# scraed/LanPaint

Measured on AMD Instinct MI355X. Metric: langevin_think_iterations_per_sec, higher is better.
Workload: dtype f32; 1 GPU; c2_sdxl: latent 1x4x128x128 per GPU, 30 sigmas x 5 think iterations, 50% box mask, stub backbone x->(0.9x,0.8x), VE/Karras schedule; rng=torch, graph=auto, mask_format=f32, mask_seen_by_kernels=bits, captured_calls=1, backbone_io=f32, replicas=1, rows_per_gpu=1, global_rows=1, latent_elements_per_gpu=65536

## Files before the change

include/lanpaint_hip.h:

```cpp
#ifndef LANPAINT_HIP_H
#define LANPAINT_HIP_H

#include <stdint.h>

#ifdef __cplusplus
extern "C" {
#endif

#define LP_ABI_VERSION 25

#define LP_API __attribute__((visibility("default")))

#define LP_OK             0
#define LP_E_INVALID     -1
#define LP_E_UNSUPPORTED -2
#define LP_E_LAUNCH      -3
#define LP_E_ALIGN       -4

#define LP_COEF_STRIDE   36
#define LP_C_SCALE        0
#define LP_C_SQRT_ABT     1
#define LP_C_OMA          2
#define LP_C_ABT          3
#define LP_C_RSIGMA       4
// ... 146 lines not shown
    int32_t      es_n_steps;
    int32_t      es_reset;
    const float* sg_sigma;
    const float* sg_schedule;
    float*       sg_times_out;
    float*       sg_scalars_out;
    int32_t*     sg_seq_out;
    uint64_t*    sg_valid_out;
    double       sg_min_step_frac;
    int32_t      sg_schedule_len, sg_seq, sg_n_steps, sg_early_stop, sg_total_steps, sg_guess;
    double*      clk_out;
    const void*  av_bits;
    float        av_frac;
    uint32_t     reserved2;
    float*       es_xte;
    uint32_t     tune;
    uint32_t     io_valid;
} lp_step_desc;
#define LP_TUNE_VEC1          (1u << 0)
#define LP_TUNE_VEC4          (1u << 1)
#define LP_TUNE_ES_NO_DECIDE  (1u << 2)
#define LP_TUNE_ES_NO_FOLD    (1u << 3)
#define LP_TUNE_ES_NO_ATOMICS (1u << 4)
#define LP_CLK_STAMPS 9

typedef struct lp_final_desc {
    int64_t   n_el;
    uint32_t  flags;
    float     cfg_scale;
    const void*  model_out;
    const void*  uncond;
    const float* y;
    const void*  mask;
    const float* x_src;
    float*       x_dst;
    float*       out;
    uint64_t*    rng_bump_ptr;
    uint64_t     rng_bump;
    const uint64_t* io_table;
} lp_final_desc;

LP_API int lp_abi_version(void);
LP_API const char* lp_strerror(int code);

LP_API int lp_coeffs(const lp_hyper* hyper, const float* ve_sigma, int ve_stride, const float* abt, int abt_stride,
              const float* replace_sigma, int rs_stride, const float* step_override, int step_stride,
              const float* t_model, int t_stride, int rows, float* coef_table, void* stream);
// ... 386 lines not shown
```

lanpaint_amd/csrc/cabi.hip:

```cpp
#include <cmath>

#include "lp_common.h"

namespace lp {
int step_dispatch(const lp_step_desc* d, hipStream_t stream, void* timer);
int replace_node_update(const lp_step_desc* d, hipGraphExec_t exec, const lp_graph_binding* b);
int timer_create(void** out);
int timer_destroy(void* h);
int timer_elapsed_ns(void* h, double* ns);
int coeffs_dispatch(const lp_hyper* h, const float* ve, int ve_stride, const float* abt, int abt_stride,
                    const float* rs, int rs_stride, const float* step_ov, int step_stride, const float* t_model,
                    int t_stride, int rows, float* table, hipStream_t stream);
int finalize_dispatch(const lp_final_desc* d, hipStream_t stream);
int sigma_times_dispatch(const float* sigma, int rows, const float* schedule, int schedule_len, int is_flow, float* times,
                         float* scalars, int32_t* seq_out, int32_t seq, hipStream_t stream);
int sigma_times_rule_dispatch(const float* sigma, int rows, const float* schedule, int schedule_len, int is_flow,
                              float* times, float* scalars, int32_t* seq_out, int32_t seq, int32_t n_steps, int32_t early_stop,
                              int32_t total_steps, double min_step_frac, int32_t guess, uint64_t* valid_out, hipStream_t stream);
int blend_dispatch(const lp_blend_desc* d, hipStream_t stream);
int philox_dispatch(float* out, int64_t n_el, uint64_t seed, uint64_t offset, uint32_t slot, hipStream_t stream);
int ring_dispatch(const float* mask, float* ring, int64_t planes, int height, int width, hipStream_t stream);
int wmse_dispatch(const float* a, const float* b, const float* mask, const float* ring, int64_t n_el, double* acc,
                  double* scratch, int scratch_blocks, hipStream_t stream);
int torch_normal_dispatch(float* out, int64_t n, uint64_t seed, uint64_t offset, uint32_t bg, hipStream_t stream);
// ... 178 lines not shown
        if (!c->graph_exec) return LP_E_INVALID;
        rc = lp::replace_node_update(c->replace, static_cast<hipGraphExec_t>(c->graph_exec), c->replace_binding);
    } else if (c->replace) {
        rc = lp::step_dispatch(c->replace, s, nullptr);
    }
    if (rc != LP_OK) return rc;
    if (c->graph_exec && hipGraphLaunch(static_cast<hipGraphExec_t>(c->graph_exec), s) != hipSuccess) return LP_E_LAUNCH;
    return c->final ? lp::finalize_dispatch(c->final, s) : LP_OK;
}

int lp_graph_bind_replace(void* graph, const lp_step_desc* captured, lp_graph_binding* out) {
    if (!graph || !captured || !out) return LP_E_INVALID;
    hipGraph_t g = static_cast<hipGraph_t>(graph);
    size_t n_root = 0;
    if (hipGraphGetRootNodes(g, nullptr, &n_root) != hipSuccess || n_root != 1) return LP_E_UNSUPPORTED;
    hipGraphNode_t root = nullptr;
    if (hipGraphGetRootNodes(g, &root, &n_root) != hipSuccess || !root) return LP_E_UNSUPPORTED;
    hipGraphNodeType ty;
    if (hipGraphNodeGetType(root, &ty) != hipSuccess || ty != hipGraphNodeTypeKernel) return LP_E_UNSUPPORTED;
    hipKernelNodeParams p{};
    if (hipGraphKernelNodeGetParams(root, &p) != hipSuccess || !p.func || !p.kernelParams) return LP_E_UNSUPPORTED;
    void* const* kp = p.kernelParams;
    const lp_step_desc* dn = static_cast<const lp_step_desc*>(kp[8]);
    if (*static_cast<void* const*>(kp[0]) != captured->x_t || *static_cast<const void* const*>(kp[2]) != captured->x ||
        !dn || dn->phases != captured->phases || !(dn->phases & LP_PH_REPLACE) || dn->n_el != captured->n_el)
        return LP_E_UNSUPPORTED;
    lp::StepPlan plan;
    const int rc = lp::plan_step(*captured, &plan);
    if (rc != LP_OK) return rc;
    if (!lp::plan_is_node(plan, p.func, p.gridDim, p.blockDim)) return LP_E_UNSUPPORTED;
    out->node = root; out->func = p.func;
    out->grid[0] = p.gridDim.x; out->grid[1] = p.gridDim.y; out->grid[2] = p.gridDim.z;
    out->block[0] = p.blockDim.x; out->block[1] = p.blockDim.y; out->block[2] = p.blockDim.z;
    out->shared_bytes = p.sharedMemBytes; out->reserved0 = 0;
    return LP_OK;
}

int lp_graph_clone_tail(void* graph, void** tail_graph_out, void** tail_exec_out) {
    if (!graph || !tail_graph_out || !tail_exec_out) return LP_E_INVALID;
    hipGraph_t clone = nullptr;
    if (hipGraphClone(&clone, static_cast<hipGraph_t>(graph)) != hipSuccess) return LP_E_LAUNCH;
    size_t n_root = 0;
    hipGraphNode_t root = nullptr;
    hipGraphExec_t exec = nullptr;
    if (hipGraphGetRootNodes(clone, nullptr, &n_root) == hipSuccess && n_root == 1 &&
        hipGraphGetRootNodes(clone, &root, &n_root) == hipSuccess && root && hipGraphDestroyNode(root) == hipSuccess &&
        hipGraphInstantiate(&exec, clone, nullptr, nullptr, 0) == hipSuccess) {
        *tail_graph_out = clone; *tail_exec_out = exec;
// ... 220 lines not shown
```

lanpaint_amd/csrc/lp_common.h:

```cpp
#pragma once
#include <hip/hip_runtime.h>
#include <hip/hip_ext.h>
#include <stdint.h>

#include "lanpaint_hip.h"

namespace lp {

constexpr int kWave = 64;

__device__ __forceinline__ int nearest_exact_index(int i, int in_size, int out_size, int rule) {
#pragma clang fp contract(off)
    const float scale = static_cast<float>(in_size) / static_cast<float>(out_size);
    const float at = static_cast<float>(i) + 0.5f;
    int s;
    if (rule == LP_NN_ATEN_SCALAR) {
        s = static_cast<int>(floorf(at * scale));
    } else {
        float src = (rule == LP_NN_ATEN_CPU_GENERIC_FMA) ? __builtin_fmaf(scale, at, -0.5f) : (scale * at - 0.5f);
        src = src < 0.0f ? 0.0f : src;
        s = static_cast<int>(floorf(static_cast<float>(static_cast<double>(src) + 0.5)));
    }
    return s < in_size - 1 ? s : in_size - 1;
}
// ... 417 lines not shown
        c[LP_C_RSCALE] = static_cast<float>(1.0 / static_cast<double>(c[LP_C_SCALE]));
    }
    const double oma_d = static_cast<double>(oma);
    float* q = c + (g ? LP_C_REGION1 : LP_C_REGION0);
    const double a = (g ? static_cast<double>(h.one_plus_lambda) : 1.0) / oma_d;
    const double dt = static_cast<double>(g ? dty : dtx);
    const double tau = s ? dt * 0.5 : dt;
    const double e = exp(-a * tau);
    const double k = -expm1(-a * tau) / a;
    const double k2 = -expm1(-2.0 * a * tau) / (2.0 * a);
    const double sd = sqrt(fmax(2.0 * k2, 0.0));
    q[s ? LP_R_E_HALF : LP_R_E_FULL] = static_cast<float>(e);
    q[s ? LP_R_K_HALF : LP_R_K_FULL] = static_cast<float>(k);
    q[s ? LP_R_STD_HALF : LP_R_STD_FULL] = static_cast<float>(sd);
    if (s == 0) {
        const double cx0 = sqrt(static_cast<double>(abt_f)) / oma_d;
        q[LP_R_DT] = static_cast<float>(dt);
        q[LP_R_A] = static_cast<float>(a);
        q[LP_R_CX0] = static_cast<float>(cx0);
        q[LP_R_CXT] = g ? static_cast<float>(a - 1.0 / oma_d) : 0.0f;
    }
}

__device__ __forceinline__ double wave_sum(double v) {
#pragma unroll
    for (int off = kWave / 2; off > 0; off >>= 1) v += __shfl_down(v, off, kWave);
    return v;
}

template <int CTRL, int ROW_MASK>
__device__ __forceinline__ float dpp_move(float v) {
    return __builtin_bit_cast(float, __builtin_amdgcn_update_dpp(0, __builtin_bit_cast(int, v), CTRL, ROW_MASK, 0xf, false));
}
template <int CTRL, int ROW_MASK>
__device__ __forceinline__ double dpp_move(double v) {
    const long long b = __builtin_bit_cast(long long, v);
    const int lo = __builtin_amdgcn_update_dpp(0, static_cast<int>(b), CTRL, ROW_MASK, 0xf, false);
    const int hi = __builtin_amdgcn_update_dpp(0, static_cast<int>(b >> 32), CTRL, ROW_MASK, 0xf, false);
    return __builtin_bit_cast(double, (static_cast<long long>(hi) << 32) | static_cast<long long>(static_cast<uint32_t>(lo)));
}
template <int CTRL, int ROW_MASK, typename T, int N>
__device__ __forceinline__ void dpp_level(T (&v)[N]) {
    T t[N];
#pragma unroll
    for (int k = 0; k < N; ++k) t[k] = dpp_move<CTRL, ROW_MASK>(v[k]);
#pragma unroll
// ... 110 lines not shown
    if (min_step_frac <= 0.0 || frac >= min_step_frac || n_steps <= 0) return n_steps;
    const double r = rint(static_cast<double>(n_steps) * frac / min_step_frac);
    return r > 0.0 ? static_cast<int32_t>(r) : 0;
}

__host__ __device__ inline int x0_dtype(uint32_t flags) {
    return (flags & LP_FL_X0_BF16) ? DT_BF16 : (flags & LP_FL_X0_F16) ? DT_F16 : DT_F32;
}
__host__ __device__ inline int xin_dtype(uint32_t flags) {
    return (flags & LP_FL_XIN_BF16) ? DT_BF16 : (flags & LP_FL_XIN_F16) ? DT_F16 : DT_F32;
}

struct StepPlan {
    const void* kernel;
    dim3 grid;
    uint32_t ph_ct;
    int vec;
    bool decide;
    int decide_slot;
    int mode, x0w, rng, es;
    bool st;
};
struct StepArgs {
    void* x_t;
    void* C;
    const void *a2, *a3, *a4, *a5;
    int32_t el_per_row;
    uint32_t flags;
    void* ptr[9];
};
int plan_step(const lp_step_desc& d, StepPlan* out, bool timed = false);
void pack_step_args(const StepPlan& p, const lp_step_desc& d, StepArgs* a);
bool plan_is_node(const StepPlan& p, const void* func, const dim3& grid, const dim3& block);

}
```

lanpaint_amd/csrc/step_kernel.hip:

```cpp
#include <cstddef>

#include "lp_common.h"

#pragma clang fp contract(off)

namespace lp {

struct RegionCoef {
    float e_full, k_full, std_full, e_half, k_half, std_half, dt, a, cx0, cxt;
};

struct RowCoef {
    float scale, sqrt_abt, oma, abt, rsigma, dtx, dty, ax, ay, dx, dy, valid;
    RegionCoef reg[2];
    float rscale;
};

__device__ __forceinline__ RowCoef load_row(const float* __restrict__ coef, int row) {
    const float* c = coef + static_cast<int64_t>(row) * LP_COEF_STRIDE;
    RowCoef r;
    r.scale = c[LP_C_SCALE]; r.sqrt_abt = c[LP_C_SQRT_ABT]; r.oma = c[LP_C_OMA]; r.abt = c[LP_C_ABT];
    r.rsigma = c[LP_C_RSIGMA]; r.dtx = c[LP_C_DTX]; r.dty = c[LP_C_DTY]; r.ax = c[LP_C_AX]; r.ay = c[LP_C_AY];
    r.dx = c[LP_C_DX]; r.dy = c[LP_C_DY]; r.valid = c[LP_C_VALID];
    r.rscale = c[LP_C_RSCALE];
// ... 212 lines not shown
    return t;
}
__device__ __forceinline__ uint64_t clk_after_loads() {
    uint64_t t;
    asm volatile("s_waitcnt vmcnt(0)\n s_memtime %0\n s_waitcnt lgkmcnt(0)" : "=s"(t)::"memory");
    return t;
}
__device__ __forceinline__ uint64_t clk_real() {
    uint64_t t;
    asm volatile("s_memrealtime %0\n s_waitcnt lgkmcnt(0)" : "=s"(t)::"memory");
    return t;
}
#define LP_CLK_DECL                                                                                                  \
    uint64_t clk_t[LP_CLK_STAMPS] = {}, clk_r0 = 0;                                                                  \
    const bool clk_on = d_arg.clk_out && threadIdx.x == 0 && blockIdx.y == 0 && (blockIdx.x == 0 || blockIdx.x == gridDim.x - 1); \
    if (clk_on) { clk_t[0] = clk_now(); clk_r0 = clk_real(); }
#define LP_CLK(k) if (clk_on) clk_t[k] = clk_now();
__device__ __forceinline__ uint64_t clk_when(uint32_t a, uint32_t b) {
    uint64_t t;
    asm volatile("s_memtime %0\n s_waitcnt lgkmcnt(0)" : "=s"(t) : "s"(a), "s"(b) : "memory");
    return t;
}
#define LP_CLK_WHEN(k, a, b) if (clk_on) clk_t[k] = clk_when(a, b);
#define LP_CLK_LOADS(k) if (clk_on) clk_t[k] = clk_after_loads();
#define LP_CLK_FLUSH                                                                                                 \
    if (clk_on) {                                                                                                    \
        double* clk_o = d_arg.clk_out + (blockIdx.x == 0 ? 0 : 16);                                                  \
        for (int k = 0; k < LP_CLK_STAMPS; ++k) clk_o[k] = clk_t[k] ? static_cast<double>(clk_t[k] - clk_t[0]) : 0.0; \
        clk_o[15] = static_cast<double>(clk_real() - clk_r0);                                                        \
        clk_o[14] = static_cast<double>(clk_r0 & 0xffffffffffffull);       \
    }
#else
#define LP_CLK_DECL
#define LP_CLK(k)
#define LP_CLK_WHEN(k, a, b)
#define LP_CLK_LOADS(k)
#define LP_CLK_FLUSH
#endif

constexpr int kBlock = 256;

constexpr uint32_t kPost = LP_PH_POST_FIRST | LP_PH_POST_STEADY;
constexpr uint32_t kTouchXt = LP_PH_REPLACE | kPost | LP_PH_PRE_HALF;

enum : int { MODE_ROW = 0, MODE_PER_EL = 1, MODE_HARD = 2 };

template <int VEC, int MODE, uint32_t PH, int X0W, int RNG, bool ST = false, int ES = 0>
__global__ __launch_bounds__(256) __attribute__((amdgpu_waves_per_eu((ES == 2 && VEC == 4 && PH != 0) ? 8 : 1))) void lp_step_kernel(void* a0, void* a1, const void* a2, const void* a3, const void* a4,
                                                       const void* a5, int32_t a_el_per_row, uint32_t a_flags,
                                                       const lp_step_desc d_arg) {
    constexpr bool PER_EL = MODE == MODE_PER_EL;
    constexpr bool HARD = MODE == MODE_HARD;
    constexpr bool SMALL = VEC == 1;
    constexpr bool PAIR = X0W == 2 && VEC == 4 && !ST;
    static_assert(!PAIR || ES == 0, "pair accesses: every lane that has not left the kernel is active");
    constexpr bool TBL = (PH & LP_PH_COEFFS) != 0 && VEC == 1;
    const unsigned el_bx = blockIdx.x - (TBL ? 1u : 0u);
    static_assert(!TBL || (!ST && !ES && (PH & LP_PH_REPLACE) != 0), "table block: the fused replace launches only");
    LP_CLK_DECL
    lp_step_desc d = d_arg;
    d.x_t = static_cast<float*>(a0); d.C = static_cast<float*>(a1);
    if constexpr ((PH & LP_PH_REPLACE) != 0) {
        d.x = static_cast<const float*>(a2);
        d.known = d.noise = static_cast<const float*>(a3);
        d.y = static_cast<const float*>(a4); d.mask = a5;
    } else {
        d.x0 = a2; d.x0_big = a3;
        if constexpr (SMALL) {
            d.coef = static_cast<const float*>(a4); d.rng_offset_ptr = static_cast<const uint64_t*>(a5);
        } else {
            d.y = static_cast<const float*>(a4); d.mask = a5;
        }
    }
    d.el_per_row = a_el_per_row; d.flags = a_flags;
    static_assert(!ES || (!ST && !PER_EL && (PH & LP_PH_REPLACE) == 0), "early stop: think-step launches of the row-table modes");
    constexpr bool es_fold = ES == 2;
    int row = blockIdx.y;
    int64_t st_base = 0, st_lo = 0, st_hi = 0;
    uint32_t st_round = 0;
    if constexpr (ST) {
        const int64_t span = 4 * static_cast<int64_t>(d.rng_bg), epr = d.el_per_row;
        const uint32_t rounds = d.rng_inc >> 2, per_round = gridDim.y / rounds;
        st_round = blockIdx.y / per_round;
        st_base = static_cast<int64_t>(st_round) * span;
        row = static_cast<int>(st_base / epr) + static_cast<int>(blockIdx.y - st_round * per_round);
        const int64_t row_lo = static_cast<int64_t>(row) * epr, row_hi = row_lo + epr;
        st_lo = row_lo > st_base ? row_lo : st_base;
        st_hi = row_hi < st_base + span ? row_hi : st_base + span;
        if (row >= d.rows || st_lo >= st_hi) return;
        const int64_t i0 = st_base + static_cast<int64_t>(blockIdx.x) * kBlock, i1 = i0 + kBlock;
        bool any = false;
#pragma unroll
        for (int k = 0; k < 4; ++k) {
            const int64_t s0 = i0 + k * static_cast<int64_t>(d.rng_bg), s1 = i1 + k * static_cast<int64_t>(d.rng_bg);
            any = any || (s0 < st_hi && s1 > st_lo);
        }
        if (!any) return;
// ... 45 lines not shown
                        for (int k = 0; k < VEC; ++k) {
                            const float sc = d.coef[static_cast<int64_t>(2 * row + static_cast<int>((nib >> k) & 1u)) * LP_COEF_STRIDE + LP_C_SCALE];
                            xo[k] = (fl & LP_FL_FLOW) ? xt[k] / sc : xt[k] * sc;
                        }
                        store_any<VEC>(d.x_in, xin_dtype(fl), i, xo);
                        return;
                    }
                }
                const float sc = load_row(d.coef, row).scale;
#pragma unroll
                for (int k = 0; k < VEC; ++k) xo[k] = (fl & LP_FL_FLOW) ? xt[k] / sc : xt[k] * sc;
                store_any<VEC>(d.x_in, xin_dtype(fl), i, xo);
                return;
            }
        }
    }
    const uint32_t ph = PH ? PH : d.phases;
    const bool flow = fl & LP_FL_FLOW;
    const bool post = ph & kPost;
    constexpr bool HOT = PH != 0 && ES == 0 && (RNG == 0 || (RNG == 1 && VEC == 1));
    constexpr bool TS = HOT && RNG == 1 && VEC == 1;
    static_assert(!TS || (!ST && (PH & LP_PH_REPLACE) == 0), "TS: think launches only");
    const bool given = HOT ? false : (fl & LP_FL_X0S_GIVEN) != 0;
    const int x0dt = X0W == 4 ? static_cast<int>(DT_F32) : x0_dtype(fl), xindt = xin_dtype(fl);
    const int64_t groups = ST ? static_cast<int64_t>(d.rng_bg) : d.el_per_row / VEC;
    const int64_t row_base = static_cast<int64_t>(row) * d.el_per_row;
    const float lam = d.lambda, opl = d.one_plus_lambda;

    RowCoef rc;
    bool av_mixed = false;
    uint32_t av_nib = 0u;
    const bool fold_coeffs = (ph & LP_PH_COEFFS) != 0;
    constexpr bool fold_sigma = (PH & LP_PH_SIGMA) != 0;
    static_assert(!fold_sigma || PH != 0, "LP_PH_SIGMA: the phase-specialised kernels only");
    auto row_times = [&](float& abt_f, float& ve_f, float& rs_f, float& tm_f) __attribute__((always_inline)) {
        if constexpr (fold_sigma) {
            float ft;
            rs_f = d.sg_sigma[row];
            sigma_to_times(rs_f, flow, ve_f, abt_f, ft);
            tm_f = flow ? ft : ve_f;
        } else {
            abt_f = d.t_abt[static_cast<int64_t>(row) * d.t_abt_stride];
            ve_f = d.t_ve ? d.t_ve[static_cast<int64_t>(row) * d.t_ve_stride] : 0.0f;
            rs_f = d.t_rsig ? d.t_rsig[static_cast<int64_t>(row) * d.t_rsig_stride] : 0.0f;
            tm_f = 0.0f;
        }
    };
    if (fold_coeffs) {
        auto build_table = [&](float abt_f, float ve_f, float rs_f, float tm_sig) __attribute__((always_inline)) {
            if (threadIdx.x < 4) {
                lp_hyper h;
                h.lambda = d.lambda; h.beta = d.beta; h.step_size = d.step_size; h.min_step_frac = d.min_step_frac;
                h.is_flow = flow ? 1 : 0; h.one_plus_lambda = d.one_plus_lambda;
                const float tm_f = fold_sigma ? tm_sig : (d.t_model ? d.t_model[static_cast<int64_t>(row) * d.t_model_stride] : 0.0f);
                const float step = d.step_size * fmaxf(1.0f - abt_f, d.min_step_frac);
                coeffs_lane(h, abt_f, ve_f, rs_f, tm_f, step, (threadIdx.x >> 1) & 1, threadIdx.x & 1,
                            d.coef_out + static_cast<int64_t>(row) * LP_COEF_STRIDE);
                if (row == 0 && threadIdx.x == 0 && d.rng_state_out) {
                    d.rng_state_out[0] = d.rng_state_val[0];
                    d.rng_state_out[1] = d.rng_state_val[1];
                }
            }
        };
        auto sigma_rule = [&]() __attribute__((always_inline)) {
            const SigmaRule rule{d.sg_n_steps, d.sg_early_stop, d.sg_total_steps, d.sg_guess, d.sg_min_step_frac, d.sg_valid_out};
            sigma_rows_and_rule(d.sg_sigma, d.rows, d.sg_schedule, d.sg_schedule_len, flow, d.sg_times_out,
                                d.sg_scalars_out, d.sg_seq_out, d.sg_seq, rule);
        };
        if constexpr (TBL) {
            if (blockIdx.x == 0) {
                if (threadIdx.x < kWave) {
                    float abt_f, ve_f, rs_f, tm_f;
                    row_times(abt_f, ve_f, rs_f, tm_f);
                    build_table(abt_f, ve_f, rs_f, tm_f);
                    LP_CLK(5)
                } else if (fold_sigma && blockIdx.y == 0 && threadIdx.x < 2 * kWave) {
                    sigma_rule();
                }
                LP_CLK(6)
                LP_CLK_FLUSH
                return;
            }
        } else {
            float abt_f, ve_f, rs_f, tm_f;
            row_times(abt_f, ve_f, rs_f, tm_f);
            if constexpr (fold_sigma) {
                if (blockIdx.x == 0 && blockIdx.y == 0 && threadIdx.x < kWave) sigma_rule();
            }
            if (blockIdx.x == 0) build_table(abt_f, ve_f, rs_f, tm_f);
            rc.scale = row_scale(flow, abt_f, ve_f);
            rc.rscale = 1.0f / rc.scale;
            rc.rsigma = rs_f;
        }
    } else {
        if constexpr (PH == 0) {
            if ((ph & LP_PH_REPLACE) && d.rng_state_out && blockIdx.x == 0 && blockIdx.y == 0 && threadIdx.x == 0) {
                d.rng_state_out[0] = d.rng_state_val[0];
                d.rng_state_out[1] = d.rng_state_val[1];
            }
        }
        if constexpr (!PER_EL) {
// ... 163 lines not shown
        constexpr bool RA = HARD && VEC == 4 && (PH & kPost) != 0;
        constexpr bool UNI = HARD && VEC == 4 && (PH & (kPost | LP_PH_PRE_HALF)) != 0 && (PH & LP_PH_REPLACE) == 0;
        constexpr bool MIXSEL = UNI && ES == 0;
        int uni = -1;
        bool need_x0 = true, need_known = true;
        bool lane_x0 = true, lane_known = true;
        bool pair_x0 = true, pair_known = true;
        if constexpr (PER_EL) {
            load_f32<VEC>(d.abt_el, i, abt_e);
            if (!flow) load_f32<VEC>(d.ve_el, i, ve_e);
        }
        if (ph & LP_PH_REPLACE) {
            load_f32<VEC>(d.x, i, xv);
            bool need_kn = true;
            if constexpr (HARD && VEC == 4 && (PH & LP_PH_REPLACE) != 0) {
                if (!(fl & LP_FL_NO_REGION_SKIP)) {
                    const uint32_t nib = (m_raw.w[0] >> (static_cast<uint32_t>(i) & 31u)) & 0xFu;
                    need_kn = __ballot(nib != 0u) != 0ull;
                }
            }
            if (!need_kn) {
#pragma unroll
                for (int k = 0; k < VEC; ++k) kn[k] = 0.0f, nv[k] = 0.0f, yv[k] = 0.0f;
            } else if (d.replace_kind == LP_REPLACE_KNOWN) {
                load_f32<VEC>(d.known, i, kn);
            } else {
                load_f32<VEC>(d.noise, i, nv);
                load_f32<VEC>(d.y, i, yv);
                if constexpr (PER_EL) load_f32<VEC>(d.rsig_el, i, rs);
            }
        } else {
            load_f32<VEC>((ES && es_gated && (ph & LP_PH_POST_STEADY)) ? d.es_xte : d.x_t, i, xt);
        }
        if ((ph & LP_PH_POST_STEADY) || ((ph & LP_PH_PRE_HALF) && !post)) load_f32<VEC>(d.C, i, cv);
        if constexpr (UNI) {
            const uint32_t nib = (m_raw.w[0] >> (static_cast<uint32_t>(i) & 31u)) & 0xFu;
            const bool any_known = __ballot(nib != 0u) != 0ull, any_inpaint = __ballot(nib != 0xFu) != 0ull;
            uni = !any_known ? 0 : (!any_inpaint ? 1 : -1);
        }
        if constexpr (RA) {
            if (!given && d.x0_big != d.x0 && !(fl & (LP_FL_CFG_FUSED | LP_FL_NO_REGION_SKIP))) {
                const uint32_t nib = (m_raw.w[0] >> (static_cast<uint32_t>(i) & 31u)) & 0xFu;
                need_known = uni != 0;
                need_x0 = uni != 1;
                lane_known = nib != 0u;
                lane_x0 = nib != 0xFu;
                if constexpr (PAIR) {
// ... 55 lines not shown
            if (post) {
                if constexpr (es_fold && VEC == 4) {
                } else if constexpr (es_fold) {
                    load_f32<VEC>(d.es_x0s[0], i, es_b0);
                    load_f32<VEC>(d.es_x0s[1], i, es_b1);
                    load_f32<VEC>(d.es_x0s[2], i, es_b2);
                } else {
                    if (es_prev >= 0) load_f32<VEC>(es_prev == 0 ? d.es_x0s[0] : es_prev == 1 ? d.es_x0s[1] : d.es_x0s[2], i, x0p);
                    if (es_anchor >= 0) load_f32<VEC>(es_anchor == 0 ? d.es_x0s[0] : es_anchor == 1 ? d.es_x0s[1] : d.es_x0s[2], i, anc);
                }
                if constexpr (!(es_fold && VEC == 4)) {
                    load_ring();
                }
            }
        }

        if constexpr (!SMALL) {
            if (need_rng && d.rng_offset_ptr) {
                rng_w0 = d.rng_offset_ptr[0];
                rng_w1 = d.rng_offset_ptr[1];
                rng_have = true;
            }
        }
        if constexpr (!TS) {
        if (d.io_table_out && el_bx == 0 && blockIdx.y == 0 && threadIdx.x == 0) {
            d.io_table_out[0] = d.io_table_val[0];
            d.io_table_out[1] = d.io_table_val[1];
            if (d.io_valid) d.io_table_out[2] = 1ull;
        }
        }
        if constexpr (PH == 0 || (PH & LP_PH_REPLACE) != 0) {
            if (d.es_reset && d.es && el_bx == 0 && blockIdx.y == 0) {
                if (d.es_partials) {
                    for (int k = threadIdx.x; k < kEsSets * kEsSlots * 8; k += kBlock) d.es_partials[k] = 0.0;
                }
                if (threadIdx.x == 0) es_reset_state(d, fold_coeffs);
            }
        }
        if constexpr (TBL) {
            float abt_f, ve_f, rs_f, tm_f;
            row_times(abt_f, ve_f, rs_f, tm_f);
            rc.scale = row_scale(flow, abt_f, ve_f);
            rc.rscale = 1.0f / rc.scale;
            rc.rsigma = rs_f;
        }

        LP_CLK(1)
        if (need_rng) {
            const bool torch_kind = RNG == 2 ? (d.rng_kind == LP_RNG_TORCH) : (RNG == 1);
            uint64_t seq = d.rng_offset, seed = d.rng_seed;
            if (rng_have) {
                seq += rng_w0;
                if (torch_kind) seed = rng_w1;
            }
            if constexpr (SMALL) {
                LP_CLK_WHEN(8, static_cast<uint32_t>(seq), static_cast<uint32_t>(seed))
            }
            if (torch_kind) {
                const bool draw_post = post && !host_post, draw_pre = (ph & LP_PH_PRE_HALF) && !host_pre;
                const uint64_t off_pre = seq + (draw_post ? d.rng_inc : 0u);
                if constexpr (ST) {
                    static_assert(!ST || VEC == 4, "the ATen layout is four elements per lane");
                    __shared__ __attribute__((aligned(16))) float st_xi[2][4][kBlock];
                    const uint32_t aten_thread = static_cast<uint32_t>(g_raw);
                    if (draw_post) {
                        float z[4];
                        torch_normal4(aten_thread, seed, seq + 4ull * st_round, z);
// ... 84 lines not shown
                }
            }
        }
        LP_CLK(4)
        const bool live = active && !es_idle;

        if (UNI && uni >= 0) {
#pragma unroll
            for (int k = 0; k < VEC; ++k) m[k] = static_cast<float>(uni);
        } else {
            cvt_mask<VEC>(mfl, i, m_raw, m);
        }
        if (post) {
            if constexpr (PAIR) {
                cvt_raw_pair(x0dt, x0_raw, x0);
                if (!(d.x0_big == d.x0 || given)) cvt_raw_pair(x0dt, x0b_raw, x0b);
            } else {
                cvt_raw<VEC>(x0dt, x0_raw, x0, i);
                if (!(d.x0_big == d.x0 || given)) cvt_raw<VEC>(x0dt, x0b_raw, x0b, i);
            }
        }

        if (ph & LP_PH_REPLACE) {
            if (d.replace_kind != LP_REPLACE_KNOWN) {
#pragma unroll
                for (int k = 0; k < VEC; ++k) {
                    const float r = PER_EL ? rs[k] : row_rsigma_of(k);
                    kn[k] = (d.replace_kind == LP_REPLACE_VE) ? fmaf(nv[k], r, yv[k])
                                                              : (r * (d.noise_scale * nv[k]) + (1.0f - r) * yv[k]);
                }
            }
#pragma unroll
            for (int k = 0; k < VEC; ++k) {
                const float xr = fmaf(kn[k], m[k], xv[k] * (1.0f - m[k]));
                float sc;
                if constexpr (PER_EL) {
                    sc = flow ? (sqrtf(abt_e[k]) + sqrtf(1.0f - abt_e[k])) : sqrtf(1.0f + ve_e[k] * ve_e[k]);
                } else {
                    sc = row_scale_of(k);
                }
                if constexpr (VEC == 4 && !PER_EL && PH != 0) {
                    xt[k] = flow ? xr * sc : div_shared(xr, sc, rc.rscale);
                } else {
                    xt[k] = flow ? xr * sc : xr / sc;
                }
            }
        }
// ... 354 lines not shown
static void plan_es(const lp_step_desc& d, StepPlan* p) {
    const bool fold = (d.flags & LP_FL_ES_GATED) && !(d.tune & LP_TUNE_ES_NO_FOLD);
    if constexpr (PH != 0) {
        if (!fold) return plan_es<VEC, MODE, 0>(d, p);
        plan_kernel<VEC, MODE, PH, X0W, RNG, false, 2>(d, p);
    } else {
        if (fold) plan_kernel<VEC, MODE, PH, X0W, RNG, false, 2>(d, p);
        else plan_kernel<VEC, MODE, PH, X0W, RNG, false, 1>(d, p);
    }
    const bool close = fold && (d.flags & LP_FL_ES_CLOSE) && d.es_index + 1 == d.es_n_steps;
    p->decide = (d.phases & kPost) && !(d.tune & LP_TUNE_ES_NO_DECIDE) && !close && (!fold || d.es_index + 1 == d.es_n_steps);
    p->decide_slot = fold ? (d.es_index & 1) : 0;
}

template <int VEC, int MODE, uint32_t PH>
static void plan_hot(const lp_step_desc& d, bool strided, bool x0_half, bool rng_torch, StepPlan* p) {
    if (strided) return x0_half ? plan_kernel<4, MODE, PH, 2, 1, true>(d, p) : plan_kernel<4, MODE, PH, 4, 1, true>(d, p);
    if (x0_half) return rng_torch ? plan_kernel<VEC, MODE, PH, 2, 1>(d, p) : plan_kernel<VEC, MODE, PH, 2, 0>(d, p);
    return rng_torch ? plan_kernel<VEC, MODE, PH, 4, 1>(d, p) : plan_kernel<VEC, MODE, PH, 4, 0>(d, p);
}

static bool aligned(const void* p, size_t a) { return p == nullptr || (reinterpret_cast<uintptr_t>(p) % a) == 0; }

template <int VEC>
static void plan_phase(const lp_step_desc& d, StepPlan* p) {
    if (d.flags & LP_FL_PER_ELEMENT) return plan_kernel<VEC, MODE_PER_EL, 0>(d, p);
    constexpr uint32_t R = LP_PH_REPLACE, F = LP_PH_POST_FIRST, S = LP_PH_POST_STEADY, P = LP_PH_PRE_HALF,
                       E = LP_PH_EMIT;
    const bool hard = (d.flags & LP_FL_MASK_BITS) && d.corr_el == nullptr;
    if (d.flags & LP_FL_AV)
        return (d.flags & LP_FL_ES) ? plan_es<VEC, MODE_ROW, 0>(d, p) : plan_kernel<VEC, MODE_ROW, 0>(d, p);
    const bool rare = (d.flags & LP_FL_X0S_GIVEN) || d.xi_post || d.xi_pre;
    const bool x0_half = x0_dtype(d.flags) != DT_F32;
    const bool pair_ok = VEC != 4 || !x0_half ||
                         (aligned(d.x0, 16) && aligned(d.x0_big, 16) && (xin_dtype(d.flags) == DT_F32 || aligned(d.x_in, 16)) &&
                          d.el_per_row % 8 == 0);
    if (d.flags & LP_FL_ES) {
        if (hard && !x0_half && !rare && (!d.es_ring || (d.flags & LP_FL_ES_RING_BITS))) {
            const bool rt = d.rng_kind == LP_RNG_TORCH;
            if (d.phases == (S | P | E))
                return rt ? plan_es<VEC, MODE_HARD, S | P | E, 4, 1>(d, p) : plan_es<VEC, MODE_HARD, S | P | E, 4, 0>(d, p);
            if (d.phases == (F | P | E))
                return rt ? plan_es<VEC, MODE_HARD, F | P | E, 4, 1>(d, p) : plan_es<VEC, MODE_HARD, F | P | E, 4, 0>(d, p);
        }
        return hard ? plan_es<VEC, MODE_HARD, 0>(d, p) : plan_es<VEC, MODE_ROW, 0>(d, p);
    }
    if (d.flags & LP_FL_MASK_U8) return plan_kernel<VEC, MODE_ROW, 0>(d, p);
    if (d.phases == (R | E | LP_PH_COEFFS))
        return hard ? plan_kernel<VEC, MODE_HARD, R | E | LP_PH_COEFFS>(d, p) : plan_kernel<VEC, MODE_ROW, R | E | LP_PH_COEFFS>(d, p);
    if (d.phases == (R | E | LP_PH_COEFFS | LP_PH_SIGMA))
        return plan_kernel<VEC, MODE_HARD, R | E | LP_PH_COEFFS | LP_PH_SIGMA>(d, p);
    const bool rng_torch = d.rng_kind == LP_RNG_TORCH;
    const bool strided = VEC == 4 && rng_torch && !d.xi_post && !d.xi_pre && d.n_el > static_cast<int64_t>(d.rng_bg) &&
                         (d.rng_bg % kBlock) == 0 &&
                         (d.rows == 1 || d.el_per_row >= 2 * static_cast<int64_t>(d.rng_bg)) && st_segments(d) != 0;
    const bool ts_rare = VEC == 1 && rng_torch && (d.n_el > static_cast<int64_t>(d.rng_bg) || d.io_table_out != nullptr);
    if (!pair_ok || rare || ts_rare) return hard ? plan_kernel<VEC, MODE_HARD, 0>(d, p) : plan_kernel<VEC, MODE_ROW, 0>(d, p);
    if (hard) {
        switch (d.phases) {
            case S | P | E: return plan_hot<VEC, MODE_HARD, S | P | E>(d, strided, x0_half, rng_torch, p);
            case F | P | E: return plan_hot<VEC, MODE_HARD, F | P | E>(d, strided, x0_half, rng_torch, p);
            case S | E: return plan_hot<VEC, MODE_HARD, S | E>(d, strided, x0_half, rng_torch, p);
            default: return plan_kernel<VEC, MODE_HARD, 0>(d, p);
        }
    }
    switch (d.phases) {
        case S | P | E: return plan_hot<VEC, MODE_ROW, S | P | E>(d, strided, x0_half, rng_torch, p);
        case F | P | E: return plan_hot<VEC, MODE_ROW, F | P | E>(d, strided, x0_half, rng_torch, p);
        case S | E: return plan_hot<VEC, MODE_ROW, S | E>(d, strided, x0_half, rng_torch, p);
        default: return plan_kernel<VEC, MODE_ROW, 0>(d, p);
    }
// ... 63 lines not shown
    } else if (d.flags & (LP_FL_ES_GATED | LP_FL_ES_CLOSE | LP_FL_ES_RING_BITS)) {
        return LP_E_INVALID;
    }

    const size_t half_al = 8, f_al = 16;
    const bool x0_half = x0_dtype(d.flags) != DT_F32, xin_half = xin_dtype(d.flags) != DT_F32;
    const bool can_vec4 = (d.el_per_row % 4 == 0) && aligned(d.x, f_al) && aligned(d.known, f_al) &&
                          aligned(d.noise, f_al) && aligned(d.y, f_al) &&
                          aligned(d.mask, (d.flags & (LP_FL_MASK_U8 | LP_FL_MASK_BITS)) ? 4 : f_al) && aligned(d.x_t, f_al) &&
                          aligned(d.C, f_al) && aligned(d.x0s, f_al) && aligned(d.x0, x0_half ? half_al : f_al) &&
                          aligned(d.x0_big, x0_half ? half_al : f_al) && aligned(d.x_in, xin_half ? half_al : f_al) &&
                          aligned(d.xi_post, f_al) && aligned(d.xi_pre, f_al) && aligned(d.abt_el, f_al) &&
                          aligned(d.ve_el, f_al) && aligned(d.rsig_el, f_al) && aligned(d.corr_el, f_al);
    bool vec4 = can_vec4 && d.n_el > 512 * 1024;
    if (d.tune & LP_TUNE_VEC4) vec4 = can_vec4;
    if (d.tune & LP_TUNE_VEC1) vec4 = false;
    if (vec4) plan_phase<4>(d, out);
    else plan_phase<1>(d, out);
    return LP_OK;
}

void pack_step_args(const StepPlan& p, const lp_step_desc& d, StepArgs* a) {
    const bool rep = (p.ph_ct & LP_PH_REPLACE) != 0, lead_y = rep || p.vec != 1;
    a->x_t = d.x_t;
    a->C = d.C;
    a->a2 = rep ? static_cast<const void*>(d.x) : d.x0;
    a->a3 = rep ? static_cast<const void*>(d.replace_kind == LP_REPLACE_KNOWN ? d.known : d.noise) : d.x0_big;
    a->a4 = lead_y ? static_cast<const void*>(d.y) : static_cast<const void*>(d.coef);
    a->a5 = lead_y ? d.mask : static_cast<const void*>(d.rng_offset_ptr);
    a->el_per_row = static_cast<int32_t>(d.el_per_row);
    a->flags = d.flags;
    void* const ptr[9] = {&a->x_t, &a->C, &a->a2, &a->a3, &a->a4, &a->a5, &a->el_per_row, &a->flags, const_cast<lp_step_desc*>(&d)};
    for (int k = 0; k < 9; ++k) a->ptr[k] = ptr[k];
}

bool plan_is_node(const StepPlan& p, const void* func, const dim3& grid, const dim3& block) {
    return !p.decide && func == p.kernel && grid.x == p.grid.x && grid.y == p.grid.y && grid.z == p.grid.z &&
           block.x == static_cast<unsigned>(kBlock) && block.y == 1 && block.z == 1;
}

#ifdef LP_TRACE_INSTANTIATIONS
}
#include <cstdio>
#include <cstdlib>
#include <mutex>
#include <set>
#include <string>
namespace lp {
struct TraceSet {
    std::mutex mu;
    std::set<std::string> seen;
    ~TraceSet() {
        const char* path = std::getenv("LANPAINT_AMD_TRACE_FILE");
        if (!path || seen.empty()) return;
        if (FILE* f = std::fopen(path, "a")) {
// ... 96 lines not shown
```

Measured before the change: 126,500 think-iterations/s.

## Split fused replace coefficient-table build across waves and pass lead times as kernel args

In the fused replace+coefficients launch with the table block, the per-row coefficient computation is split across four waves: separate lanes compute the exp, expm1 and sqrt terms in double, and one lane writes the header. This replaces a single wave doing all of it serially. The leading time values (abt/sigma, ve/rsig) are passed through the x_t/C argument slots and read as scalar constant loads, with how to read them encoded in private flag bits. This is meant to shorten the critical path of the table block, which sits on the serial dependency chain of each step. The cost is more complex argument packing, a plan restriction on table strides, and extra clock stamps for profiling.

```diff
diff --git a/include/lanpaint_hip.h b/include/lanpaint_hip.h
--- a/include/lanpaint_hip.h
+++ b/include/lanpaint_hip.h
@@ -192,7 +192,7 @@
 #define LP_TUNE_ES_NO_DECIDE  (1u << 2)
 #define LP_TUNE_ES_NO_FOLD    (1u << 3)
 #define LP_TUNE_ES_NO_ATOMICS (1u << 4)
-#define LP_CLK_STAMPS 9
+#define LP_CLK_STAMPS 12
 
 typedef struct lp_final_desc {
     int64_t   n_el;
diff --git a/lanpaint_amd/csrc/cabi.hip b/lanpaint_amd/csrc/cabi.hip
--- a/lanpaint_amd/csrc/cabi.hip
+++ b/lanpaint_amd/csrc/cabi.hip
@@ -224,8 +224,8 @@
     if (hipGraphKernelNodeGetParams(root, &p) != hipSuccess || !p.func || !p.kernelParams) return LP_E_UNSUPPORTED;
     void* const* kp = p.kernelParams;
     const lp_step_desc* dn = static_cast<const lp_step_desc*>(kp[8]);
-    if (*static_cast<void* const*>(kp[0]) != captured->x_t || *static_cast<const void* const*>(kp[2]) != captured->x ||
-        !dn || dn->phases != captured->phases || !(dn->phases & LP_PH_REPLACE) || dn->n_el != captured->n_el)
+    if (!dn || dn->x_t != captured->x_t || dn->x != captured->x || dn->phases != captured->phases ||
+        !(dn->phases & LP_PH_REPLACE) || dn->n_el != captured->n_el)
         return LP_E_UNSUPPORTED;
     lp::StepPlan plan;
     const int rc = lp::plan_step(*captured, &plan);
diff --git a/lanpaint_amd/csrc/lp_common.h b/lanpaint_amd/csrc/lp_common.h
--- a/lanpaint_amd/csrc/lp_common.h
+++ b/lanpaint_amd/csrc/lp_common.h
@@ -463,6 +463,64 @@
     }
 }
 
+__device__ __forceinline__ void coeffs_header(const lp_hyper& h, float abt_f, float ve_f, float rs_f, float tm_f, float step,
+                                              float* __restrict__ c) {
+#pragma clang fp contract(off)
+    const float oma = 1.0f - abt_f;
+    const float dtx2 = 2.0f * step * 1.0f, dty2 = 2.0f * step * h.beta;
+    const float dtx = dtx2 / 2.0f, dty = dty2 / 2.0f;
+    const float atx = (1.0f / oma) * dtx2 / 2.0f;
+    const float aty = (h.one_plus_lambda / oma) * dty2 / 2.0f;
+    const bool valid = step > 0.0f;
+    const float scale = row_scale(h.is_flow, abt_f, ve_f);
+    c[LP_C_SCALE] = scale;
+    c[LP_C_SQRT_ABT] = sqrtf(abt_f);
+    c[LP_C_OMA] = oma;
+    c[LP_C_ABT] = abt_f;
+    c[LP_C_RSIGMA] = rs_f;
+    c[LP_C_DTX] = dtx;
+    c[LP_C_DTY] = dty;
+    c[LP_C_AX] = atx / dtx;
+    c[LP_C_AY] = aty / dty;
+    c[LP_C_DX] = sqrtf(2.0f);
+    c[LP_C_DY] = sqrtf(2.0f);
+    c[LP_C_VALID] = valid ? 1.0f : 0.0f;
+    c[LP_C_TMODEL] = tm_f;
+    c[LP_C_RSCALE] = static_cast<float>(1.0 / static_cast<double>(scale));
+}
+
+enum : int { LP_TV_E = 0, LP_TV_K = 1, LP_TV_SD = 2, LP_TV_EXTRAS = 3 };
+
+__device__ __forceinline__ void coeffs_value(const lp_hyper& h, float abt_f, float step, int g, int s, int what,
+                                             float* __restrict__ c) {
+#pragma clang fp contract(off)
+    const float oma = 1.0f - abt_f;
+    const float dtx2 = 2.0f * step * 1.0f, dty2 = 2.0f * step * h.beta;
+    const float dtx = dtx2 / 2.0f, dty = dty2 / 2.0f;
+    const double oma_d = static_cast<double>(oma);
+    float* q = c + (g ? LP_C_REGION1 : LP_C_REGION0);
+    const double a = (g ? static_cast<double>(h.one_plus_lambda) : 1.0) / oma_d;
+    const double dt = static_cast<double>(g ? dty : dtx);
+    const double tau = s ? dt * 0.5 : dt;
+    if (what == LP_TV_E) {
+        const double e = exp(-a * tau);
+        q[s ? LP_R_E_HALF : LP_R_E_FULL] = static_cast<float>(e);
+    } else if (what == LP_TV_K) {
+        const double k = -expm1(-a * tau) / a;
+        q[s ? LP_R_K_HALF : LP_R_K_FULL] = static_cast<float>(k);
+    } else if (what == LP_TV_SD) {
+        const double k2 = -expm1(-2.0 * a * tau) / (2.0 * a);
+        const double sd = sqrt(fmax(2.0 * k2, 0.0));
+        q[s ? LP_R_STD_HALF : LP_R_STD_FULL] = static_cast<float>(sd);
+    } else {
+        const double cx0 = sqrt(static_cast<double>(abt_f)) / oma_d;
+        q[LP_R_DT] = static_cast<float>(dt);
+        q[LP_R_A] = static_cast<float>(a);
+        q[LP_R_CX0] = static_cast<float>(cx0);
+        q[LP_R_CXT] = g ? static_cast<float>(a - 1.0 / oma_d) : 0.0f;
+    }
+}
+
 __device__ __forceinline__ double wave_sum(double v) {
 #pragma unroll
     for (int off = kWave / 2; off > 0; off >>= 1) v += __shfl_down(v, off, kWave);
@@ -619,9 +677,7 @@
     bool st;
 };
 struct StepArgs {
-    void* x_t;
-    void* C;
-    const void *a2, *a3, *a4, *a5;
+    const void *a0, *a1, *a2, *a3, *a4, *a5;
     int32_t el_per_row;
     uint32_t flags;
     void* ptr[9];
diff --git a/lanpaint_amd/csrc/step_kernel.hip b/lanpaint_amd/csrc/step_kernel.hip
--- a/lanpaint_amd/csrc/step_kernel.hip
+++ b/lanpaint_amd/csrc/step_kernel.hip
@@ -258,6 +258,12 @@
     return t;
 }
 #define LP_CLK_WHEN(k, a, b) if (clk_on) clk_t[k] = clk_when(a, b);
+__device__ __forceinline__ uint64_t clk_behind(float a, float b) {
+    uint64_t t;
+    asm volatile("s_memtime %0\n s_waitcnt lgkmcnt(0)" : "=s"(t) : "v"(a), "v"(b) : "memory");
+    return t;
+}
+#define LP_CLK_BEHIND(k, a, b) if (clk_on) clk_t[k] = clk_behind(a, b);
 #define LP_CLK_LOADS(k) if (clk_on) clk_t[k] = clk_after_loads();
 #define LP_CLK_FLUSH                                                                                                 \
     if (clk_on) {                                                                                                    \
@@ -270,6 +276,7 @@
 #define LP_CLK_DECL
 #define LP_CLK(k)
 #define LP_CLK_WHEN(k, a, b)
+#define LP_CLK_BEHIND(k, a, b)
 #define LP_CLK_LOADS(k)
 #define LP_CLK_FLUSH
 #endif
@@ -277,6 +284,22 @@
 constexpr int kBlock = 256;
 
 constexpr uint32_t kPost = LP_PH_POST_FIRST | LP_PH_POST_STEADY;
+
+constexpr uint32_t kArgRsIsVe = 1u << 26;
+constexpr uint32_t kArgKnown = 1u << 27;
+constexpr int kArgLead0 = 28, kArgLead1 = 30;
+constexpr uint32_t kArgPrivate = 0xFC000000u;
+enum : uint32_t { LEAD_ROW0 = 0, LEAD_ROW = 1, LEAD_NULL = 2 };
+
+__device__ __forceinline__ float lead_time(const void* p, const void* safe, uint32_t how, int row) {
+    typedef const __attribute__((address_space(4))) float* const_time;
+    return ((const_time)(how == LEAD_NULL ? safe : p))[how == LEAD_ROW ? row : 0];
+}
+__device__ __forceinline__ float lead_value(float loaded, uint32_t how) { return how == LEAD_NULL ? 0.0f : loaded; }
+__device__ __forceinline__ float const_time_at(const float* p, int64_t i) {
+    typedef const __attribute__((address_space(4))) float* const_time;
+    return ((const_time)p)[i];
+}
 constexpr uint32_t kTouchXt = LP_PH_REPLACE | kPost | LP_PH_PRE_HALF;
 
 enum : int { MODE_ROW = 0, MODE_PER_EL = 1, MODE_HARD = 2 };
@@ -295,7 +318,9 @@
     static_assert(!TBL || (!ST && !ES && (PH & LP_PH_REPLACE) != 0), "table block: the fused replace launches only");
     LP_CLK_DECL
     lp_step_desc d = d_arg;
-    d.x_t = static_cast<float*>(a0); d.C = static_cast<float*>(a1);
+    if constexpr (!TBL) {
+        d.x_t = static_cast<float*>(a0); d.C = static_cast<float*>(a1);
+    }
     if constexpr ((PH & LP_PH_REPLACE) != 0) {
         d.x = static_cast<const float*>(a2);
         d.known = d.noise = static_cast<const float*>(a3);
@@ -308,7 +333,7 @@
             d.y = static_cast<const float*>(a4); d.mask = a5;
         }
     }
-    d.el_per_row = a_el_per_row; d.flags = a_flags;
+    d.el_per_row = a_el_per_row; d.flags = TBL ? (a_flags & ~kArgPrivate) : a_flags;
     static_assert(!ES || (!ST && !PER_EL && (PH & LP_PH_REPLACE) == 0), "early stop: think-step launches of the row-table modes");
     constexpr bool es_fold = ES == 2;
     int row = blockIdx.y;
@@ -400,6 +425,10 @@
     constexpr bool TS = HOT && RNG == 1 && VEC == 1;
     static_assert(!TS || (!ST && (PH & LP_PH_REPLACE) == 0), "TS: think launches only");
     const bool given = HOT ? false : (fl & LP_FL_X0S_GIVEN) != 0;
+    auto rep_known = [&]() __attribute__((always_inline)) -> bool {
+        if constexpr (TBL) return (a_flags & kArgKnown) != 0;
+        else return d.replace_kind == LP_REPLACE_KNOWN;
+    };
     const int x0dt = X0W == 4 ? static_cast<int>(DT_F32) : x0_dtype(fl), xindt = xin_dtype(fl);
     const int64_t groups = ST ? static_cast<int64_t>(d.rng_bg) : d.el_per_row / VEC;
     const int64_t row_base = static_cast<int64_t>(row) * d.el_per_row;
@@ -411,12 +440,25 @@
     const bool fold_coeffs = (ph & LP_PH_COEFFS) != 0;
     constexpr bool fold_sigma = (PH & LP_PH_SIGMA) != 0;
     static_assert(!fold_sigma || PH != 0, "LP_PH_SIGMA: the phase-specialised kernels only");
+    float lead0 = 0.0f, lead1 = 0.0f;
+    if constexpr (TBL) {
+        lead0 = lead_time(a0, a2, (a_flags >> kArgLead0) & 3u, row);
+        if constexpr (!fold_sigma) lead1 = lead_time(a1, a2, a_flags >> kArgLead1, row);
+    }
     auto row_times = [&](float& abt_f, float& ve_f, float& rs_f, float& tm_f) __attribute__((always_inline)) {
         if constexpr (fold_sigma) {
             float ft;
-            rs_f = d.sg_sigma[row];
+            rs_f = TBL ? lead0 : d.sg_sigma[row];
             sigma_to_times(rs_f, flow, ve_f, abt_f, ft);
             tm_f = flow ? ft : ve_f;
+        } else if constexpr (TBL) {
+            abt_f = lead0;
+            const float l1 = lead_value(lead1, a_flags >> kArgLead1);
+            const float ve_d = (flow && d.t_ve) ? const_time_at(d.t_ve, static_cast<int64_t>(row) * d.t_ve_stride) : 0.0f;
+            const float rs_d = (a_flags & kArgRsIsVe) ? l1 : (!flow && d.t_rsig) ? const_time_at(d.t_rsig, static_cast<int64_t>(row) * d.t_rsig_stride) : 0.0f;
+            ve_f = flow ? ve_d : l1;
+            rs_f = flow ? l1 : rs_d;
+            tm_f = 0.0f;
         } else {
             abt_f = d.t_abt[static_cast<int64_t>(row) * d.t_abt_stride];
             ve_f = d.t_ve ? d.t_ve[static_cast<int64_t>(row) * d.t_ve_stride] : 0.0f;
@@ -447,14 +489,55 @@
         };
         if constexpr (TBL) {
             if (blockIdx.x == 0) {
-                if (threadIdx.x < kWave) {
-                    float abt_f, ve_f, rs_f, tm_f;
-                    row_times(abt_f, ve_f, rs_f, tm_f);
-                    build_table(abt_f, ve_f, rs_f, tm_f);
-                    LP_CLK(5)
-                } else if (fold_sigma && blockIdx.y == 0 && threadIdx.x < 2 * kWave) {
-                    sigma_rule();
-                }
+                const unsigned wave = threadIdx.x / kWave, lane = threadIdx.x % kWave;
+                const bool rule = fold_sigma && blockIdx.y == 0;
+                if (wave == 1) {
+                    if (rule) {
+                        asm volatile("" ::"s"(reinterpret_cast<uintptr_t>(d.sg_schedule)), "s"(d.sg_schedule_len), "s"(d.rows),
+                                     "s"(reinterpret_cast<uintptr_t>(d.sg_times_out)), "s"(reinterpret_cast<uintptr_t>(d.sg_scalars_out)),
+                                     "s"(reinterpret_cast<uintptr_t>(d.sg_seq_out)), "s"(d.sg_seq), "s"(d.sg_n_steps), "s"(d.sg_early_stop),
+                                     "s"(d.sg_total_steps), "s"(d.sg_guess), "s"(d.sg_min_step_frac),
+                                     "s"(reinterpret_cast<uintptr_t>(d.sg_valid_out)), "s"(reinterpret_cast<uintptr_t>(d.rng_state_out)),
+                                     "s"(d.rng_state_val[0]), "s"(d.rng_state_val[1]));
+                    }
+                    if (row == 0 && lane == 0 && d.rng_state_out) {
+                        d.rng_state_out[0] = d.rng_state_val[0];
+                        d.rng_state_out[1] = d.rng_state_val[1];
+                    }
+                    if (rule) sigma_rule();
+                }
+                if (wave != 1 || !rule) {
+                    asm volatile("" ::"s"(lead0), "s"(lead1), "s"(d.lambda), "s"(d.beta), "s"(d.step_size), "s"(d.min_step_frac),
+                                 "s"(d.one_plus_lambda), "s"(reinterpret_cast<uintptr_t>(d.coef_out)),
+                                 "s"(reinterpret_cast<uintptr_t>(d.t_ve)), "s"(d.t_ve_stride),
+                                 "s"(reinterpret_cast<uintptr_t>(d.t_rsig)), "s"(d.t_rsig_stride),
+                                 "s"(reinterpret_cast<uintptr_t>(d.t_model)), "s"(d.t_model_stride));
+                    LP_CLK(9)
+                    LP_CLK_WHEN(10, __float_as_uint(lead0), __float_as_uint(lead1))
+                    float abt_f, ve_f, rs_f, tm_sig;
+                    row_times(abt_f, ve_f, rs_f, tm_sig);
+                    const float tm_f = fold_sigma ? tm_sig
+                                                  : (d.t_model ? const_time_at(d.t_model, static_cast<int64_t>(row) * d.t_model_stride) : 0.0f);
+                    lp_hyper h;
+                    h.lambda = d.lambda; h.beta = d.beta; h.step_size = d.step_size; h.min_step_frac = d.min_step_frac;
+                    h.is_flow = flow ? 1 : 0; h.one_plus_lambda = d.one_plus_lambda;
+                    const float step = d.step_size * fmaxf(1.0f - abt_f, d.min_step_frac);
+                    float* const crow = d.coef_out + static_cast<int64_t>(row) * LP_COEF_STRIDE;
+                    const int g = (lane >> 1) & 1, s = lane & 1;
+                    if (wave == 0) {
+                        if (lane < 4) coeffs_value(h, abt_f, step, g, s, LP_TV_E, crow);
+                        else if (lane < 6) coeffs_value(h, abt_f, step, lane & 1, 0, LP_TV_EXTRAS, crow);
+                        LP_CLK(5)
+                    } else if (wave == 2) {
+                        if (lane < 4) coeffs_value(h, abt_f, step, g, s, LP_TV_K, crow);
+                    } else if (wave == 3) {
+                        if (lane < 4) coeffs_value(h, abt_f, step, g, s, LP_TV_SD, crow);
+                    }
+                    if (wave == (rule ? 2u : 1u) && lane == 0) coeffs_header(h, abt_f, ve_f, rs_f, tm_f, step, crow);
+                }
+#ifdef LP_SHADER_CLOCK
+                __syncthreads();
+#endif
                 LP_CLK(6)
                 LP_CLK_FLUSH
                 return;
@@ -664,7 +747,7 @@
             if (!need_kn) {
 #pragma unroll
                 for (int k = 0; k < VEC; ++k) kn[k] = 0.0f, nv[k] = 0.0f, yv[k] = 0.0f;
-            } else if (d.replace_kind == LP_REPLACE_KNOWN) {
+            } else if (rep_known()) {
                 load_f32<VEC>(d.known, i, kn);
             } else {
                 load_f32<VEC>(d.noise, i, nv);
@@ -766,6 +849,13 @@
                 rng_have = true;
             }
         }
+        if constexpr (TBL) {
+            asm volatile("" ::"s"(lead0), "s"(lead1), "s"(reinterpret_cast<uintptr_t>(d.x_t)), "s"(reinterpret_cast<uintptr_t>(d.x_in)),
+                         "s"(d.replace_kind), "s"(d.noise_scale), "s"(reinterpret_cast<uintptr_t>(d.t_ve)), "s"(d.t_ve_stride),
+                         "s"(reinterpret_cast<uintptr_t>(d.t_rsig)), "s"(d.t_rsig_stride),
+                         "s"(reinterpret_cast<uintptr_t>(d.io_table_out)), "s"(d.io_table_val[0]), "s"(d.io_table_val[1]),
+                         "s"(d.io_valid), "s"(d.es_reset));
+        }
         if constexpr (!TS) {
         if (d.io_table_out && el_bx == 0 && blockIdx.y == 0 && threadIdx.x == 0) {
             d.io_table_out[0] = d.io_table_val[0];
@@ -787,6 +877,7 @@
             rc.scale = row_scale(flow, abt_f, ve_f);
             rc.rscale = 1.0f / rc.scale;
             rc.rsigma = rs_f;
+            LP_CLK_BEHIND(11, rc.rscale, rc.rsigma)
         }
 
         LP_CLK(1)
@@ -917,7 +1008,7 @@
         }
 
         if (ph & LP_PH_REPLACE) {
-            if (d.replace_kind != LP_REPLACE_KNOWN) {
+            if (!rep_known()) {
 #pragma unroll
                 for (int k = 0; k < VEC; ++k) {
                     const float r = PER_EL ? rs[k] : row_rsigma_of(k);
@@ -1318,6 +1409,11 @@
 
 static bool aligned(const void* p, size_t a) { return p == nullptr || (reinterpret_cast<uintptr_t>(p) % a) == 0; }
 
+static bool lead_strides_ok(const lp_step_desc& d) {
+    auto ok = [](const void* t, int32_t stride) { return !t || stride == 0 || stride == 1; };
+    return ok(d.t_abt, d.t_abt_stride) && ok(d.t_ve, d.t_ve_stride) && ok(d.t_rsig, d.t_rsig_stride);
+}
+
 template <int VEC>
 static void plan_phase(const lp_step_desc& d, StepPlan* p) {
     if (d.flags & LP_FL_PER_ELEMENT) return plan_kernel<VEC, MODE_PER_EL, 0>(d, p);
@@ -1342,7 +1438,7 @@
         return hard ? plan_es<VEC, MODE_HARD, 0>(d, p) : plan_es<VEC, MODE_ROW, 0>(d, p);
     }
     if (d.flags & LP_FL_MASK_U8) return plan_kernel<VEC, MODE_ROW, 0>(d, p);
-    if (d.phases == (R | E | LP_PH_COEFFS))
+    if (d.phases == (R | E | LP_PH_COEFFS) && (VEC != 1 || lead_strides_ok(d)))
         return hard ? plan_kernel<VEC, MODE_HARD, R | E | LP_PH_COEFFS>(d, p) : plan_kernel<VEC, MODE_ROW, R | E | LP_PH_COEFFS>(d, p);
     if (d.phases == (R | E | LP_PH_COEFFS | LP_PH_SIGMA))
         return plan_kernel<VEC, MODE_HARD, R | E | LP_PH_COEFFS | LP_PH_SIGMA>(d, p);
@@ -1452,15 +1548,29 @@
 
 void pack_step_args(const StepPlan& p, const lp_step_desc& d, StepArgs* a) {
     const bool rep = (p.ph_ct & LP_PH_REPLACE) != 0, lead_y = rep || p.vec != 1;
-    a->x_t = d.x_t;
-    a->C = d.C;
+    const bool tbl = (p.ph_ct & LP_PH_COEFFS) != 0 && p.vec == 1;
+    a->a0 = d.x_t;
+    a->a1 = d.C;
+    a->flags = d.flags;
+    if (tbl) {
+        const bool sig = (p.ph_ct & LP_PH_SIGMA) != 0, flow = (d.flags & LP_FL_FLOW) != 0;
+        auto how = [](const void* t, int32_t stride) -> uint32_t {
+            return !t ? LEAD_NULL : stride == 0 ? LEAD_ROW0 : LEAD_ROW;
+        };
+        a->a0 = sig ? d.sg_sigma : d.t_abt;
+        a->a1 = sig ? nullptr : (flow ? d.t_rsig : d.t_ve);
+        const uint32_t h0 = sig ? LEAD_ROW : how(d.t_abt, d.t_abt_stride);
+        const uint32_t h1 = sig ? LEAD_NULL : (flow ? how(d.t_rsig, d.t_rsig_stride) : how(d.t_ve, d.t_ve_stride));
+        const bool rs_is_ve = !sig && !flow && d.t_rsig && d.t_rsig == d.t_ve && d.t_rsig_stride == d.t_ve_stride;
+        a->flags = (d.flags & ~kArgPrivate) | (h0 << kArgLead0) | (h1 << kArgLead1) |
+                   (d.replace_kind == LP_REPLACE_KNOWN ? kArgKnown : 0u) | (rs_is_ve ? kArgRsIsVe : 0u);
+    }
     a->a2 = rep ? static_cast<const void*>(d.x) : d.x0;
     a->a3 = rep ? static_cast<const void*>(d.replace_kind == LP_REPLACE_KNOWN ? d.known : d.noise) : d.x0_big;
     a->a4 = lead_y ? static_cast<const void*>(d.y) : static_cast<const void*>(d.coef);
     a->a5 = lead_y ? d.mask : static_cast<const void*>(d.rng_offset_ptr);
     a->el_per_row = static_cast<int32_t>(d.el_per_row);
-    a->flags = d.flags;
-    void* const ptr[9] = {&a->x_t, &a->C, &a->a2, &a->a3, &a->a4, &a->a5, &a->el_per_row, &a->flags, const_cast<lp_step_desc*>(&d)};
+    void* const ptr[9] = {&a->a0, &a->a1, &a->a2, &a->a3, &a->a4, &a->a5, &a->el_per_row, &a->flags, const_cast<lp_step_desc*>(&d)};
     for (int k = 0; k < 9; ++k) a->ptr[k] = ptr[k];
 }
 
```

New measurement: 127,000 think-iterations/s (median of 2 runs). Within noise of the previous version (+0.4%).
